# 30stomercury/whisper-char-alignment

Hardware: AMD Instinct MI355X
Metric: utterances/sec (whisper-medium, 10s audio, char align) at 1/2/4/8 MI355X (higher is better)
Workload: dtype f16x2 (hi + lo operand pairs on the f16 MFMA pipe: fp32-equivalent operands, fp32 accumulate)

## Files before the change

### whisper-char-alignment_amd/csrc/attention_split.hip

```cpp
#include <cstdlib>

#include "attn_common.h"
#include "launch.h"

namespace wca {

namespace {

template <bool CAUSAL, bool CAPTURE>
__global__ __launch_bounds__(256, 2) void attn_split_kernel(AttnArgs a) {
  constexpr int NW = 4;
  extern __shared__ __attribute__((aligned(16))) char smem[];
  half_t* lds = reinterpret_cast<half_t*>(smem);
  const int tid = threadIdx.x;
  const int lane = tid & 63;
  const int wave = __builtin_amdgcn_readfirstlane(tid >> 6);
  const int fr = lane & 15, fg = lane >> 4;
  constexpr int QB = NW * 32;
  const int n_qt = (a.nq + QB - 1) / QB;
  const int lid = xcd_remap(blockIdx.x, n_qt * a.H * a.B);
  const int bh = lid / n_qt;
  const int b = bh / a.H, h = bh - b * a.H;
  const int q_blk = (lid - bh * n_qt) * QB;
  const int q_wave = q_blk + wave * 32;

  half8 qh[2][2], ql[2][2];
  int qrow[2];
#pragma unroll
  for (int sub = 0; sub < 2; ++sub) {
    qrow[sub] = q_wave + sub * 16 + fr;
    const int qc = qrow[sub] < a.nq ? qrow[sub] : a.nq - 1;
    const half_t* qp = a.Q + (long)b * a.q_bs + (long)qc * a.q_rs + h * 64 + fg * 8;
    qh[sub][0] = *reinterpret_cast<const half8*>(qp);
    qh[sub][1] = *reinterpret_cast<const half8*>(qp + 32);
    ql[sub][0] = *reinterpret_cast<const half8*>(qp + a.q_lo);
    ql[sub][1] = *reinterpret_cast<const half8*>(qp + a.q_lo + 32);
  }
  const float c_log2 = a.scale * LOG2E;
  constexpr bool PRE = !CAPTURE;
  if (PRE) {
#pragma unroll
    for (int sub = 0; sub < 2; ++sub)
#pragma unroll
      for (int ks = 0; ks < 2; ++ks)
#pragma unroll
        for (int j = 0; j < 8; ++j) {
          const HalfPair pr = split_pair(((float)qh[sub][ks][j] + (float)ql[sub][ks][j]) * c_log2);
          qh[sub][ks][j] = pr.hi;
          ql[sub][ks][j] = pr.lo;
        }
  }
  const float cm = PRE ? 1.0f : c_log2;

  int nk_eff = a.nk;
  if (CAUSAL) {
    const int qhi = q_blk + QB;
    nk_eff = qhi < a.nk ? qhi : a.nk;
  }
  const int nkt = (nk_eff + KT - 1) / KT;

  const half_t* Kb = a.K + (long)b * a.k_bs + h * 64;
  const half_t* Vb = a.V + (long)b * a.v_bs + h * 64;

  auto stage = [&](int buf, int kt) {
    half_t* Kh = lds + buf * (4 * TILE);
    half_t* Kl = Kh + TILE;
    half_t* Vh = Kl + TILE;
    half_t* Vl = Vh + TILE;
#pragma unroll
    for (int i = 0; i < (8 + NW - 1) / NW; ++i) {
      const int piece = wave + NW * i;
      if (piece >= 8) break;
      const int rbase = piece * 8;
      const int r = rbase + (lane >> 3);
      int key = kt * KT + r;
      key = key < a.nk ? key : a.nk - 1;
      const int ck = (lane & 7) ^ swz128(r);
      const int cv = (lane & 7) ^ (r & 6);
      const half_t* kp = Kb + (long)key * a.k_rs + ck * 8;
      const half_t* vp = Vb + (long)key * a.v_rs + cv * 8;
      glds16(kp, Kh + rbase * 64);
      glds16(kp + a.k_lo, Kl + rbase * 64);
      glds16(vp, Vh + rbase * 64);
      glds16(vp + a.v_lo, Vl + rbase * 64);
    }
  };

  f32x4 ot[2][4];
#pragma unroll
  for (int s = 0; s < 2; ++s)
#pragma unroll
    for (int d = 0; d < 4; ++d) ot[s][d] = f32x4{0.f, 0.f, 0.f, 0.f};
  unsigned vaddr[4];
  {
    const int qd = fr >> 2, pd = fr & 3;
    const int swz = (4 * (fg & 1)) | (qd & 2);
#pragma unroll
    for (int dt = 0; dt < 4; ++dt)
      vaddr[dt] = lds_off(lds) + 2u * (unsigned)((4 * fg + qd) * 64 + (((2 * dt + (pd >> 1)) ^ swz) << 3) + 4 * (pd & 1));
  }
  unsigned kaddr[2][4];
#pragma unroll
  for (int ks = 0; ks < 2; ++ks)
#pragma unroll
    for (int t = 0; t < 4; ++t) {
      const int r = t * 16 + fr;
      kaddr[ks][t] = lds_off(lds) + 2u * (unsigned)(r * 64 + (((ks * 4 + fg) ^ swz128(r)) << 3));
    }
  float m_run[2] = {-INFINITY, -INFINITY};
  float l_part[2] = {0.f, 0.f};

  stage(0, 0);
  for (int kt = 0; kt < nkt; ++kt) {
    wait_vm0();
    __builtin_amdgcn_s_barrier();
    asm volatile("" ::: "memory");
    if (kt + 1 < nkt) stage((kt + 1) & 1, kt + 1);
    f32x4 st[2][4];
#pragma unroll
    for (int s = 0; s < 2; ++s)
#pragma unroll
      for (int t = 0; t < 4; ++t) st[s][t] = f32x4{0.f, 0.f, 0.f, 0.f};
    {
      constexpr int KLO = TILE * (int)sizeof(half_t);
      const unsigned sbk = (unsigned)(kt & 1) * (unsigned)(4 * TILE * sizeof(half_t));
      half8 kh[2][4], kl[2][4];
#pragma unroll
      for (int ks = 0; ks < 2; ++ks) {
#pragma unroll
        for (int t = 0; t < 4; ++t) kl[ks][t] = lds_read_b128_asm<KLO>(kaddr[ks][t] + sbk);
#pragma unroll
        for (int t = 0; t < 4; ++t) kh[ks][t] = lds_read_b128_asm<0>(kaddr[ks][t] + sbk);
      }
      WCA_LGKM_WAIT4(12, kl[0][0], kl[0][1], kl[0][2], kl[0][3]);
#pragma unroll
      for (int s = 0; s < 2; ++s)
#pragma unroll
        for (int t = 0; t < 4; ++t) st[s][t] = __builtin_amdgcn_mfma_f32_16x16x32_f16(kl[0][t], qh[s][0], st[s][t], 0, 0, 0);
      WCA_LGKM_WAIT4(8, kh[0][0], kh[0][1], kh[0][2], kh[0][3]);
#pragma unroll
      for (int s = 0; s < 2; ++s)
#pragma unroll
        for (int t = 0; t < 4; ++t) st[s][t] = __builtin_amdgcn_mfma_f32_16x16x32_f16(kh[0][t], ql[s][0], st[s][t], 0, 0, 0);
#pragma unroll
      for (int s = 0; s < 2; ++s)
#pragma unroll
        for (int t = 0; t < 4; ++t) st[s][t] = __builtin_amdgcn_mfma_f32_16x16x32_f16(kh[0][t], qh[s][0], st[s][t], 0, 0, 0);
      WCA_LGKM_WAIT4(4, kl[1][0], kl[1][1], kl[1][2], kl[1][3]);
#pragma unroll
      for (int s = 0; s < 2; ++s)
#pragma unroll
        for (int t = 0; t < 4; ++t) st[s][t] = __builtin_amdgcn_mfma_f32_16x16x32_f16(kl[1][t], qh[s][1], st[s][t], 0, 0, 0);
      WCA_LGKM_WAIT4(0, kh[1][0], kh[1][1], kh[1][2], kh[1][3]);
#pragma unroll
      for (int s = 0; s < 2; ++s)
#pragma unroll
        for (int t = 0; t < 4; ++t) st[s][t] = __builtin_amdgcn_mfma_f32_16x16x32_f16(kh[1][t], ql[s][1], st[s][t], 0, 0, 0);
#pragma unroll
      for (int s = 0; s < 2; ++s)
#pragma unroll
        for (int t = 0; t < 4; ++t) st[s][t] = __builtin_amdgcn_mfma_f32_16x16x32_f16(kh[1][t], qh[s][1], st[s][t], 0, 0, 0);
    }

    if (CAPTURE) {
#pragma unroll
      for (int s = 0; s < 2; ++s) {
        if (qrow[s] < a.nq) {
#pragma unroll
          for (int t = 0; t < 4; ++t) {
            const int key4 = kt * KT + t * 16 + 4 * fg;
            if (key4 < a.cap_cols) {
              float* cp = a.cap + (long)b * a.cap_bs + (long)h * a.cap_hs + (long)qrow[s] * a.cap_ld + key4;
              const f32x4 lg = st[s][t] * a.scale;
              if (key4 + 4 <= a.cap_cols) {
                *reinterpret_cast<f32x4*>(cp) = lg;
              } else {
#pragma unroll
                for (int r = 0; r < 3; ++r)
                  if (key4 + r < a.cap_cols) cp[r] = lg[r];
              }
            }
          }
        }
      }
    }
    const bool tail_tile = (kt * KT + KT > a.nk);
    const bool diag_tile = CAUSAL && (kt * KT + KT - 1 > q_wave);
    if (tail_tile || diag_tile) {
#pragma unroll
      for (int s = 0; s < 2; ++s)
#pragma unroll
        for (int t = 0; t < 4; ++t)
#pragma unroll
          for (int r = 0; r < 4; ++r) {
            const int key = kt * KT + t * 16 + 4 * fg + r;
            bool dead = key >= a.nk;
            if (CAUSAL) dead = dead || (key > qrow[s]);
            st[s][t][r] = dead ? -INFINITY : st[s][t][r];
          }
    }
    float mx[2];
#pragma unroll
    for (int s = 0; s < 2; ++s) {
      float m = fmaxf(fmaxf(st[s][0][0], st[s][0][1]), fmaxf(st[s][0][2], st[s][0][3]));
#pragma unroll
      for (int t = 1; t < 4; ++t) {
        m = fmaxf(fmaxf(m, st[s][t][0]), st[s][t][1]);
        m = fmaxf(fmaxf(m, st[s][t][2]), st[s][t][3]);
      }
      mx[s] = xor32_max(xor16_max(m));
    }
    const float thr_raw = 8.0f / cm;
    if (__any((mx[0] > m_run[0] + thr_raw) || (mx[1] > m_run[1] + thr_raw) || (m_run[0] == -INFINITY && mx[0] != -INFINITY) ||
              (m_run[1] == -INFINITY && mx[1] != -INFINITY))) {
#pragma unroll
      for (int s = 0; s < 2; ++s) {
        const float m_new = fmaxf(m_run[s], mx[s]);
        const float alpha = (m_run[s] == -INFINITY) ? 1.0f : __builtin_amdgcn_exp2f((m_run[s] - m_new) * cm);
        l_part[s] *= alpha;
#pragma unroll
        for (int d = 0; d < 4; ++d) ot[s][d] *= alpha;
        m_run[s] = m_new;
      }
    }
    half8 ph[2][2], pl[2][2];
#pragma unroll
    for (int s = 0; s < 2; ++s) {
      const float mref = (m_run[s] == -INFINITY) ? 0.f : m_run[s];
      const f32x2 mm = f32x2{mref, mref};
      f32x2 psum2 = f32x2{0.f, 0.f};
#pragma unroll
      for (int k2 = 0; k2 < 2; ++k2) {
        half2_ hh[4], ll[4];
#pragma unroll
        for (int u = 0; u < 4; ++u) {
          const int t = 2 * k2 + (u >> 1), r0 = 2 * (u & 1);
          f32x2 x = f32x2{st[s][t][r0], st[s][t][r0 + 1]} - mm;
          if (!PRE) x = x * f32x2{cm, cm};
          const f32x2 p = f32x2{__builtin_amdgcn_exp2f(x[0]), __builtin_amdgcn_exp2f(x[1])};
          psum2 += p;
          hh[u] = __builtin_convertvector(p, half2_);
          {
            const unsigned hu = __builtin_bit_cast(unsigned, hh[u]);
            unsigned lu;
            asm("v_fma_mixlo_f16 %0, %1, 1.0, -%2 op_sel:[0,0,0] op_sel_hi:[0,0,1]" : "=v"(lu) : "v"(p[0]), "v"(hu));
            asm("v_fma_mixhi_f16 %0, %1, 1.0, -%2 op_sel:[0,0,1] op_sel_hi:[0,0,1]" : "+v"(lu) : "v"(p[1]), "v"(hu));
            ll[u] = __builtin_bit_cast(half2_, lu);
          }
        }
        ph[s][k2] = half8{hh[0][0], hh[0][1], hh[1][0], hh[1][1], hh[2][0], hh[2][1], hh[3][0], hh[3][1]};
        pl[s][k2] = half8{ll[0][0], ll[0][1], ll[1][0], ll[1][1], ll[2][0], ll[2][1], ll[3][0], ll[3][1]};
      }
      l_part[s] += psum2[0] + psum2[1];
    }

    {
      const unsigned sb = (unsigned)(kt & 1) * (unsigned)(4 * TILE * sizeof(half_t));
      constexpr int VH = 2 * TILE * (int)sizeof(half_t), VL = 3 * TILE * (int)sizeof(half_t);
      constexpr int K2 = 32 * 64 * (int)sizeof(half_t), B16 = 16 * 64 * (int)sizeof(half_t);
      half4 c_[8], n_[8];
#define WCA_ISSUE_V(R, A)                                                                    \
  do {                                                                                       \
    R[0] = lds_read_tr_asm<VH>(A);                                                               \
    R[1] = lds_read_tr_asm<VH + B16>(A);                                                         \
    R[2] = lds_read_tr_asm<VL>(A);                                                               \
    R[3] = lds_read_tr_asm<VL + B16>(A);                                                         \
    R[4] = lds_read_tr_asm<VH + K2>(A);                                                          \
    R[5] = lds_read_tr_asm<VH + K2 + B16>(A);                                                    \
    R[6] = lds_read_tr_asm<VL + K2>(A);                                                          \
    R[7] = lds_read_tr_asm<VL + K2 + B16>(A);                                                    \
  } while (0)
      WCA_ISSUE_V(c_, vaddr[0] + sb);
#pragma unroll
      for (int dt = 0; dt < 4; ++dt) {
        if (dt < 3) {
          WCA_ISSUE_V(n_, vaddr[dt + 1] + sb);
          WCA_LGKM_WAIT8(8, c_[0], c_[1], c_[2], c_[3], c_[4], c_[5], c_[6], c_[7]);
        } else {
          WCA_LGKM_WAIT8(0, c_[0], c_[1], c_[2], c_[3], c_[4], c_[5], c_[6], c_[7]);
        }
#pragma unroll
        for (int k2 = 0; k2 < 2; ++k2) {
          const half8 vh = __builtin_shufflevector(c_[4 * k2], c_[4 * k2 + 1], 0, 1, 2, 3, 4, 5, 6, 7);
          const half8 vl = __builtin_shufflevector(c_[4 * k2 + 2], c_[4 * k2 + 3], 0, 1, 2, 3, 4, 5, 6, 7);
#pragma unroll
          for (int s = 0; s < 2; ++s) {
            ot[s][dt] = __builtin_amdgcn_mfma_f32_16x16x32_f16(vl, ph[s][k2], ot[s][dt], 0, 0, 0);
            ot[s][dt] = __builtin_amdgcn_mfma_f32_16x16x32_f16(vh, pl[s][k2], ot[s][dt], 0, 0, 0);
            ot[s][dt] = __builtin_amdgcn_mfma_f32_16x16x32_f16(vh, ph[s][k2], ot[s][dt], 0, 0, 0);
          }
        }
        if (dt < 3) {
#pragma unroll
          for (int i = 0; i < 8; ++i) c_[i] = n_[i];
        }
      }
#undef WCA_ISSUE_V
    }
  }

#pragma unroll
  for (int s = 0; s < 2; ++s) {
    const float l = xor32_sum(xor16_sum(l_part[s]));
    if (qrow[s] >= a.nq) continue;
    const float inv = 1.0f / l;
    half_t* op = a.O + (long)b * a.o_bs + (long)qrow[s] * a.o_rs + h * 64 + 4 * fg;
#pragma unroll
    for (int dt = 0; dt < 4; ++dt) {
      half4 oh, ol;
#pragma unroll
      for (int r = 0; r < 4; ++r) {
        const HalfPair pr = split_pair(ot[s][dt][r] * inv);
        oh[r] = pr.hi;
        ol[r] = pr.lo;
      }
      *reinterpret_cast<half4*>(op + dt * 16) = oh;
      *reinterpret_cast<half4*>(op + a.o_lo + dt * 16) = ol;
    }
  }
}



#define WCA_S_PIN8(A, B, C, D, E, F, G, H) asm volatile("" : "+v"(A), "+v"(B), "+v"(C), "+v"(D), "+v"(E), "+v"(F), "+v"(G), "+v"(H)::"memory")

template <int DROP>
__global__ __launch_bounds__(256, 2) void attn_split32_kernel(AttnArgs a) {
  constexpr int NW = 4;
  extern __shared__ __attribute__((aligned(16))) char smem[];
  half_t* lds = reinterpret_cast<half_t*>(smem);
  const int tid = threadIdx.x;
  const int lane = tid & 63;
  const int wave = __builtin_amdgcn_readfirstlane(tid >> 6);
  const int l31 = lane & 31, hh = lane >> 5;
  constexpr int QB = NW * 32;
  constexpr int TB = TILE * (int)sizeof(half_t);
  constexpr int SLOT_BYTES = 4 * TB;
  const int n_qt = (a.nq + QB - 1) / QB;
  const int lid = xcd_remap(blockIdx.x, n_qt * a.H * a.B);
  const int bh = lid / n_qt;
  const int b = bh / a.H, h = bh - b * a.H;
  const int q_wave = (lid - bh * n_qt) * QB + wave * 32;
  const int qrow = q_wave + l31;
  const float c_log2 = a.scale * LOG2E;
  half8 qh[4], ql[4];
  {
    const int qc = qrow < a.nq ? qrow : a.nq - 1;
    const half_t* qp = a.Q + (long)b * a.q_bs + (long)qc * a.q_rs + h * 64 + hh * 8;
#pragma unroll
    for (int ks = 0; ks < 4; ++ks) {
      const half8 rh = *reinterpret_cast<const half8*>(qp + ks * 16);
      const half8 rl = *reinterpret_cast<const half8*>(qp + a.q_lo + ks * 16);
#pragma unroll
      for (int j = 0; j < 8; ++j) {
        const HalfPair pr = split_pair(((float)rh[j] + (float)rl[j]) * c_log2);
        qh[ks][j] = pr.hi;
        ql[ks][j] = pr.lo;
      }
    }
  }
  const int nkt = (a.nk + KT - 1) / KT;
  const int kbytes = (int)(((long)(a.nk - 1) * a.k_rs + 64) * 2), vbytes = (int)(((long)(a.nk - 1) * a.v_rs + 64) * 2);
  const half_t* Kb = a.K + (long)b * a.k_bs + h * 64;
  const half_t* Vb = a.V + (long)b * a.v_bs + h * 64;
  const __amdgpu_buffer_rsrc_t rkh = __builtin_amdgcn_make_buffer_rsrc(const_cast<half_t*>(Kb), 0, kbytes, 0x00020000);
  const __amdgpu_buffer_rsrc_t rkl = __builtin_amdgcn_make_buffer_rsrc(const_cast<half_t*>(Kb + a.k_lo), 0, kbytes, 0x00020000);
  const __amdgpu_buffer_rsrc_t rvh = __builtin_amdgcn_make_buffer_rsrc(const_cast<half_t*>(Vb), 0, vbytes, 0x00020000);
  const __amdgpu_buffer_rsrc_t rvl = __builtin_amdgcn_make_buffer_rsrc(const_cast<half_t*>(Vb + a.v_lo), 0, vbytes, 0x00020000);
  unsigned dk[2], dv[2];
#pragma unroll
  for (int i = 0; i < 2; ++i) {
    const int r = (wave * 2 + i) * 8 + (lane >> 3);
    dk[i] = (unsigned)(r * a.k_rs * 2 + (((lane & 7) ^ ((r >> 1) & 7)) << 4));
    dv[i] = (unsigned)(r * a.v_rs * 2 + (((lane & 7) ^ ((r & 2) << 1)) << 4));
  }
  const unsigned k_tile_bytes = (unsigned)(KT * a.k_rs * 2), v_tile_bytes = (unsigned)(KT * a.v_rs * 2);
  auto stage = [&](int buf, int kt) {
    half_t* Kh = lds + buf * (4 * TILE);
#pragma unroll
    for (int i = 0; i < 2; ++i) {
      const int rbase = (wave * 2 + i) * 8;
      __builtin_amdgcn_raw_ptr_buffer_load_lds(rkh, (WCA_LDS void*)(Kh + rbase * 64), 16, (int)dk[i], (int)(kt * k_tile_bytes), 0, 0);
      __builtin_amdgcn_raw_ptr_buffer_load_lds(rkl, (WCA_LDS void*)(Kh + TILE + rbase * 64), 16, (int)dk[i], (int)(kt * k_tile_bytes), 0, 0);
      __builtin_amdgcn_raw_ptr_buffer_load_lds(rvh, (WCA_LDS void*)(Kh + 2 * TILE + rbase * 64), 16, (int)dv[i], (int)(kt * v_tile_bytes), 0, 0);
      __builtin_amdgcn_raw_ptr_buffer_load_lds(rvl, (WCA_LDS void*)(Kh + 3 * TILE + rbase * 64), 16, (int)dv[i], (int)(kt * v_tile_bytes), 0, 0);
    }
  };

  const int kswz = (l31 >> 1) & 7;
  const unsigned lds_base = lds_off(lds);
  unsigned ka[4];
#pragma unroll
  for (int ks = 0; ks < 4; ++ks) ka[ks] = lds_base + (unsigned)(l31 * 128 + 16 * ((hh ^ kswz) & 1) + 32 * (ks ^ (kswz >> 1)));
  const int vq = (lane & 15) >> 2, vp = lane & 3, vg1 = (lane >> 4) & 1;
  const int vkey0 = 4 * hh + vq;
  const int vdim0 = 16 * vg1 + 4 * vp;
  const int vsw = (vkey0 & 2) << 1;
  unsigned va[2];
#pragma unroll
  for (int db = 0; db < 2; ++db)
    va[db] = lds_base + (unsigned)(2 * TB + vkey0 * 128 + (((4 * db + (vdim0 >> 3)) ^ vsw) << 4) + 2 * (vdim0 & 7));

  f32x16 ot[2];
#pragma unroll
  for (int d = 0; d < 2; ++d)
#pragma unroll
    for (int r = 0; r < 16; ++r) ot[d][r] = 0.f;
  float m_run = -INFINITY;
  float l_run = 0.f;
  f32x16 cinit;
#pragma unroll
  for (int r = 0; r < 16; ++r) cinit[r] = 0.f;

  stage(0, 0);
  auto tile = [&](auto slot_c, int kt) {
    constexpr int SLOT = decltype(slot_c)::value;
    constexpr int SB = SLOT * SLOT_BYTES;
    asm volatile("s_waitcnt vmcnt(0)" ::: "memory");
    __builtin_amdgcn_s_barrier();
    asm volatile("" ::: "memory");
    if (kt + 1 < nkt) stage(SLOT ^ 1, kt + 1);

    f32x16 st[2];
    {
      half8 kl0[4], kh0[4], kl1[4], kh1[4];
      kl0[0] = lds_read_b128_asm<SB + TB>(ka[0]);
      kl0[1] = lds_read_b128_asm<SB + TB>(ka[1]);
      kl0[2] = lds_read_b128_asm<SB + TB>(ka[2]);
      kl0[3] = lds_read_b128_asm<SB + TB>(ka[3]);
      kh0[0] = lds_read_b128_asm<SB>(ka[0]);
      kh0[1] = lds_read_b128_asm<SB>(ka[1]);
      kh0[2] = lds_read_b128_asm<SB>(ka[2]);
      kh0[3] = lds_read_b128_asm<SB>(ka[3]);
      kl1[0] = lds_read_b128_asm<SB + TB + 32 * 128>(ka[0]);
      kl1[1] = lds_read_b128_asm<SB + TB + 32 * 128>(ka[1]);
      kl1[2] = lds_read_b128_asm<SB + TB + 32 * 128>(ka[2]);
      kl1[3] = lds_read_b128_asm<SB + TB + 32 * 128>(ka[3]);
      kh1[0] = lds_read_b128_asm<SB + 32 * 128>(ka[0]);
      kh1[1] = lds_read_b128_asm<SB + 32 * 128>(ka[1]);
      kh1[2] = lds_read_b128_asm<SB + 32 * 128>(ka[2]);
      kh1[3] = lds_read_b128_asm<SB + 32 * 128>(ka[3]);
      if constexpr (DROP == 0) {
      WCA_LGKM_WAIT4(12, kl0[0], kl0[1], kl0[2], kl0[3]);
      st[0] = __builtin_amdgcn_mfma_f32_32x32x16_f16(kl0[0], qh[0], cinit, 0, 0, 0);
#pragma unroll
      for (int ks = 1; ks < 4; ++ks) st[0] = __builtin_amdgcn_mfma_f32_32x32x16_f16(kl0[ks], qh[ks], st[0], 0, 0, 0);
      WCA_LGKM_WAIT4(8, kh0[0], kh0[1], kh0[2], kh0[3]);
#pragma unroll
      for (int ks = 0; ks < 4; ++ks) st[0] = __builtin_amdgcn_mfma_f32_32x32x16_f16(kh0[ks], ql[ks], st[0], 0, 0, 0);
#pragma unroll
      for (int ks = 0; ks < 4; ++ks) st[0] = __builtin_amdgcn_mfma_f32_32x32x16_f16(kh0[ks], qh[ks], st[0], 0, 0, 0);
      WCA_LGKM_WAIT4(4, kl1[0], kl1[1], kl1[2], kl1[3]);
// ... 37 lines not shown
    P##hb[1] = lds_read_tr_asm<SB + 1 * 2048 + 1024>(va[DB]);              \
    P##ha[2] = lds_read_tr_asm<SB + 2 * 2048>(va[DB]);                     \
    P##hb[2] = lds_read_tr_asm<SB + 2 * 2048 + 1024>(va[DB]);              \
    P##ha[3] = lds_read_tr_asm<SB + 3 * 2048>(va[DB]);                     \
    P##hb[3] = lds_read_tr_asm<SB + 3 * 2048 + 1024>(va[DB]);              \
    P##la[0] = lds_read_tr_asm<SB + TB + 0 * 2048>(va[DB]);                \
    P##lb[0] = lds_read_tr_asm<SB + TB + 0 * 2048 + 1024>(va[DB]);         \
    P##la[1] = lds_read_tr_asm<SB + TB + 1 * 2048>(va[DB]);                \
    P##lb[1] = lds_read_tr_asm<SB + TB + 1 * 2048 + 1024>(va[DB]);         \
    P##la[2] = lds_read_tr_asm<SB + TB + 2 * 2048>(va[DB]);                \
    P##lb[2] = lds_read_tr_asm<SB + TB + 2 * 2048 + 1024>(va[DB]);         \
    P##la[3] = lds_read_tr_asm<SB + TB + 3 * 2048>(va[DB]);                \
    P##lb[3] = lds_read_tr_asm<SB + TB + 3 * 2048 + 1024>(va[DB]);         \
  } while (0)
    WCA_ISSUE_V32(v0, 0);
    if (kt * KT + KT > a.nk) {
#pragma unroll
      for (int kb = 0; kb < 2; ++kb)
#pragma unroll
        for (int r = 0; r < 16; ++r) {
          const int key = kt * KT + kb * 32 + (r & 3) + 8 * (r >> 2) + 4 * hh;
          st[kb][r] = key >= a.nk ? -INFINITY : st[kb][r];
        }
    }
    float mx;
    {
      float m0 = max3f(st[0][0], st[0][1], st[0][2]), m1 = max3f(st[0][3], st[0][4], st[0][5]);
      float m2 = max3f(st[0][6], st[0][7], st[0][8]), m3 = max3f(st[0][9], st[0][10], st[0][11]);
      m0 = max3f(m0, st[0][12], st[0][13]);
      m1 = max3f(m1, st[0][14], st[0][15]);
      m2 = max3f(m2, st[1][0], st[1][1]);
      m3 = max3f(m3, st[1][2], st[1][3]);
      m0 = max3f(m0, st[1][4], st[1][5]);
      m1 = max3f(m1, st[1][6], st[1][7]);
      m2 = max3f(m2, st[1][8], st[1][9]);
      m3 = max3f(m3, st[1][10], st[1][11]);
      m0 = max3f(m0, st[1][12], st[1][13]);
      m1 = max3f(m1, st[1][14], st[1][15]);
      mx = fmaxf(max3f(m0, m1, m2), m3);
      mx = xor32_max(mx);
    }
    if (__any((mx > RESCALE_THR) || (m_run == -INFINITY && mx != -INFINITY))) {
      const float m_eff = (m_run == -INFINITY) ? 0.f : m_run;
      const float m_new = fmaxf(m_run, mx + m_eff);
      const float delta = (m_new == -INFINITY) ? 0.f : m_new - m_eff;
      const float alpha = (m_run == -INFINITY) ? 1.0f : __builtin_amdgcn_exp2f(m_run - m_new);
      l_run *= alpha;
#pragma unroll
      for (int d = 0; d < 2; ++d)
#pragma unroll
        for (int r = 0; r < 16; ++r) ot[d][r] *= alpha;
#pragma unroll
      for (int kb = 0; kb < 2; ++kb)
#pragma unroll
        for (int r = 0; r < 16; ++r) st[kb][r] -= delta;
      m_run = m_new;
      const float c0 = (m_new != -INFINITY) ? -m_new : 0.f;
#pragma unroll
      for (int r = 0; r < 16; ++r) cinit[r] = c0;
    }
    half8 ph[4], pl[4];
    {
      f32x2 psum = f32x2{0.f, 0.f};
#pragma unroll
      for (int s4 = 0; s4 < 4; ++s4) {
        half2_ hq[4], lq[4];
#pragma unroll
        for (int u = 0; u < 4; ++u) {
          const int r0 = 8 * (s4 & 1) + 2 * u;
          const f32x2 p = f32x2{__builtin_amdgcn_exp2f(st[s4 >> 1][r0]), __builtin_amdgcn_exp2f(st[s4 >> 1][r0 + 1])};
          psum += p;
          hq[u] = __builtin_convertvector(p, half2_);
          const unsigned hu = __builtin_bit_cast(unsigned, hq[u]);
          unsigned lu;
          asm("v_fma_mixlo_f16 %0, %1, 1.0, -%2 op_sel:[0,0,0] op_sel_hi:[0,0,1]" : "=v"(lu) : "v"(p[0]), "v"(hu));
          asm("v_fma_mixhi_f16 %0, %1, 1.0, -%2 op_sel:[0,0,1] op_sel_hi:[0,0,1]" : "+v"(lu) : "v"(p[1]), "v"(hu));
          lq[u] = __builtin_bit_cast(half2_, lu);
        }
        ph[s4] = half8{hq[0][0], hq[0][1], hq[1][0], hq[1][1], hq[2][0], hq[2][1], hq[3][0], hq[3][1]};
        pl[s4] = half8{lq[0][0], lq[0][1], lq[1][0], lq[1][1], lq[2][0], lq[2][1], lq[3][0], lq[3][1]};
      }
      l_run += psum[0] + psum[1];
    }
    WCA_LGKM_WAIT8(0, v0ha[0], v0hb[0], v0ha[1], v0hb[1], v0ha[2], v0hb[2], v0ha[3], v0hb[3]);
    WCA_S_PIN8(v0la[0], v0lb[0], v0la[1], v0lb[1], v0la[2], v0lb[2], v0la[3], v0lb[3]);
    WCA_ISSUE_V32(v1, 1);
#pragma unroll
    for (int s4 = 0; s4 < 4; ++s4) {
      const half8 wh = __builtin_shufflevector(v0ha[s4], v0hb[s4], 0, 1, 2, 3, 4, 5, 6, 7);
      const half8 wl = __builtin_shufflevector(v0la[s4], v0lb[s4], 0, 1, 2, 3, 4, 5, 6, 7);
      if (!(DROP & 4)) ot[0] = __builtin_amdgcn_mfma_f32_32x32x16_f16(wl, ph[s4], ot[0], 0, 0, 0);
      if (!(DROP & 8)) ot[0] = __builtin_amdgcn_mfma_f32_32x32x16_f16(wh, pl[s4], ot[0], 0, 0, 0);
      ot[0] = __builtin_amdgcn_mfma_f32_32x32x16_f16(wh, ph[s4], ot[0], 0, 0, 0);
    }
    WCA_LGKM_WAIT8(0, v1ha[0], v1hb[0], v1ha[1], v1hb[1], v1ha[2], v1hb[2], v1ha[3], v1hb[3]);
    WCA_S_PIN8(v1la[0], v1lb[0], v1la[1], v1lb[1], v1la[2], v1lb[2], v1la[3], v1lb[3]);
#pragma unroll
    for (int s4 = 0; s4 < 4; ++s4) {
      const half8 wh = __builtin_shufflevector(v1ha[s4], v1hb[s4], 0, 1, 2, 3, 4, 5, 6, 7);
      const half8 wl = __builtin_shufflevector(v1la[s4], v1lb[s4], 0, 1, 2, 3, 4, 5, 6, 7);
      if (!(DROP & 4)) ot[1] = __builtin_amdgcn_mfma_f32_32x32x16_f16(wl, ph[s4], ot[1], 0, 0, 0);
      if (!(DROP & 8)) ot[1] = __builtin_amdgcn_mfma_f32_32x32x16_f16(wh, pl[s4], ot[1], 0, 0, 0);
      ot[1] = __builtin_amdgcn_mfma_f32_32x32x16_f16(wh, ph[s4], ot[1], 0, 0, 0);
    }
#undef WCA_ISSUE_V32
  };
  for (int kt = 0; kt < nkt; kt += 2) {
    tile(IntC<0>{}, kt);
    if (kt + 1 < nkt) tile(IntC<1>{}, kt + 1);
  }

  const float inv = 1.0f / xor32_sum(l_run);
  half_t* op = a.O + (long)b * a.o_bs + (long)qrow * a.o_rs + h * 64;
#pragma unroll
  for (int db = 0; db < 2; ++db)
#pragma unroll
    for (int g2 = 0; g2 < 2; ++g2) {
      unsigned wh[2][2], wl[2][2];
#pragma unroll
      for (int e = 0; e < 2; ++e)
#pragma unroll
        for (int k2 = 0; k2 < 2; ++k2) {
          const Half2Pair pr = split_pair2(ot[db][4 * (2 * g2 + e) + 2 * k2] * inv, ot[db][4 * (2 * g2 + e) + 2 * k2 + 1] * inv);
          wh[e][k2] = __builtin_bit_cast(unsigned, pr.hi);
          wl[e][k2] = __builtin_bit_cast(unsigned, pr.lo);
        }
      typedef unsigned u32x4 __attribute__((ext_vector_type(4)));
      u32x4 oh, ol;
      {
        auto r0 = __builtin_amdgcn_permlane32_swap(wh[0][0], wh[1][0], false, false);
        auto r1 = __builtin_amdgcn_permlane32_swap(wh[0][1], wh[1][1], false, false);
        oh = u32x4{r0[0], r1[0], r0[1], r1[1]};
        auto s0 = __builtin_amdgcn_permlane32_swap(wl[0][0], wl[1][0], false, false);
        auto s1 = __builtin_amdgcn_permlane32_swap(wl[0][1], wl[1][1], false, false);
        ol = u32x4{s0[0], s1[0], s0[1], s1[1]};
      }
      if (qrow < a.nq) {
        *reinterpret_cast<u32x4*>(op + 32 * db + 16 * g2 + 8 * hh) = oh;
        *reinterpret_cast<u32x4*>(op + a.o_lo + 32 * db + 16 * g2 + 8 * hh) = ol;
      }
    }
}

}

hipError_t launch_attention_split(const AttnArgs& a, hipStream_t s) {
  if (a.nq <= 0 || a.B <= 0) return hipSuccess;
  if (!attn_args_ok(a)) return hipErrorInvalidValue;
  if ((a.q_lo % 8) || (a.k_lo % 8) || (a.v_lo % 8) || (a.o_lo % 4) || a.q_lo <= 0 || a.k_lo <= 0 || a.v_lo <= 0 || a.o_lo <= 0) return hipErrorInvalidValue;
  const bool cap = a.cap != nullptr && a.cap_cols > 0;
  constexpr int LDS = 2 * 4 * TILE * (int)sizeof(half_t);
  const dim3 grid(((a.nq + 127) / 128) * a.H * a.B), block(256);
  const int variant = a.variant ? a.variant : debug_switch(DBG_ATTN_SPLIT_VARIANT);
  if (!a.causal && !cap && a.nq >= 64 && variant != 1 && (a.o_rs % 8) == 0 && (a.o_lo % 8) == 0) {
    auto launch32 = [&](auto drop_c) { return launch_lds<attn_split32_kernel<decltype(drop_c)::value>, LDS>(grid, block, LDS, s, a); };
    switch (debug_switch(DBG_ATTN_SPLIT_DROP)) {
      case 0: return launch32(IntC<0>{});
      case 1: return launch32(IntC<1>{});
      case 2: return launch32(IntC<2>{});
      case 3: return launch32(IntC<3>{});
      case 4: return launch32(IntC<4>{});
      case 8: return launch32(IntC<8>{});
      case 9: return launch32(IntC<9>{});
      case 12: return launch32(IntC<12>{});
      case 15: return launch32(IntC<15>{});
      default: return hipErrorInvalidValue;
    }
  }
  if (a.causal) {
    if (cap) return launch_lds<attn_split_kernel<true, true>, LDS>(grid, block, LDS, s, a);
    return launch_lds<attn_split_kernel<true, false>, LDS>(grid, block, LDS, s, a);
  }
  if (cap) return launch_lds<attn_split_kernel<false, true>, LDS>(grid, block, LDS, s, a);
  return launch_lds<attn_split_kernel<false, false>, LDS>(grid, block, LDS, s, a);
}

}
```

### whisper-char-alignment_amd/csrc/engine_forward.hip

```cpp
#include "engine_internal.h"

using namespace wca;

namespace wca {

hipError_t gemm(wca_engine* e, hipStream_t s, Gemm g) {
  if (g.c_lo > 0 && g.out_mode == 0) g.out_mode = 4;
  if (g.w_plain != nullptr && use_wlo(e) && e->wlo_bases.count(g.w_plain)) {
    GemmArgs x = flat(g.A, g.lda, g.w_lo ? g.w_lo : wlo_of(e, g.w_plain), g.k_plain, g.C, g.ldc, g.M, g.N, g.k_plain);
    x.a_rows_per_batch = g.a_rows_per_batch;
    x.a_batch_stride = g.a_batch_stride;
    x.site = g.site;
    x.out_mode = 2;
    if (g.out_mode != 2) {
      GrowBuf& tmp = e->wlo_tmp[s == e->stream ? 0 : 1];
      if (hipError_t he = tmp.ensure((size_t)g.M * g.N * sizeof(float)); he != hipSuccess) return he;
      x.C = tmp.p;
      x.ldc = g.N;
      x.out_mode = 1;
      g.addend = (const float*)tmp.p;
      g.ld_addend = g.N;
    }
    if (hipError_t he = launch_gemm(x, s); he != hipSuccess) return he;
  }
// ... 190 lines not shown
  Gemm g = flat(e->xn, sp, e->kv_w, e->sw.kv_w, d, kvbuf, (sp ? 2 : 1) * L * 2 * dt, B * N_CTX, n_cols);
  g.bias = e->kv_b;
  g.c_lo = sp ? (long)L * 2 * dt : 0;
  g.site = 3;
  HIPCHK(gemm(e, e->stream, g));
  return WCA_OK;
}

struct DecPass {
  hipStream_t s;
  int B, nq;
  bool pair;
  const half_t* kv;
  int kv_group;
  half_t* cache;
  int T_max;
  StepPos pos;
  const int* nk_rows() const { return pos.rows ? pos.rows + B : nullptr; }
  half_t* scatter;
  float* cap;
  int Fpad, Fcap;
  int l0, l1;
  bool stop_at_capture;
};

namespace {

int dec_linear(wca_engine* e, const DecPass& p, Gemm g, const half_t* W2, half_t* xn) {
  if (!p.pair) return dec_gemm(e, p.s, g, xn);
  const bool f16_out = g.out_mode == 0;
  if (g.A32) {
    HIPCHK(launch_layernorm_f16(g.A32, g.ln_gamma, g.ln_beta, xn, g.M, g.K, 1e-5f, p.s, 2 * g.K, g.K));
    g.A = xn;
  }
  Gemm m = flat(g.A, true, g.W, W2, g.K, g.C, (f16_out ? 2 : 1) * g.ldc, g.M, g.N);
  m.bias = g.bias;
  m.gelu = g.gelu;
  m.out_mode = g.out_mode;
  m.site = g.site;
  m.c_lo = f16_out ? g.N : 0;
  m.sk_part = e->sk_big[1];
  m.sk_bytes = e->sk_big_bytes;
  HIPCHK(gemm(e, p.s, m));
  return WCA_OK;
}

Gemm dec_flat(const half_t* A, const half_t* W, const float* bias, void* C, int M, int N, int K) {
  Gemm g = flat(A, K, W, K, C, N, M, N, K);
  g.bias = bias;
  g.site = 2;
  return g;
}
Gemm dec_flat_ln(const float* x, const float* gamma, const float* beta, const half_t* W, const float* bias, void* C, int M, int N, int K) {
  Gemm g = flat(nullptr, 0, W, K, C, N, M, N, K);
  g.A32 = x;
  g.ln_gamma = gamma;
  g.ln_beta = beta;
  g.bias = bias;
  g.site = 2;
  return g;
}

AttnArgs attn_common(const wca_engine* e, const DecPass& p, const half_t* q, int q_rs, half_t* o) {
  const int dt = e->dims.n_text_state, H = e->dims.n_text_head, om = p.pair ? 2 : 1;
  AttnArgs a{};
  a.Q = q;
  a.q_bs = (long)p.nq * q_rs;
  a.q_rs = q_rs;
  a.O = o;
  a.o_bs = (long)p.nq * om * dt;
  a.o_rs = om * dt;
  if (p.pair) {
    a.split = 1;
    a.o_lo = dt;
  }
  a.nq = p.nq;
  a.H = H;
  a.B = p.B;
  a.scale = 1.0f / std::sqrt((float)(dt / H));
  return a;
}

AttnArgs self_attn_args(const wca_engine* e, const DecPass& p, const half_t* qkv, half_t* o, const half_t* kc, const half_t* vc) {
  const int dt = e->dims.n_text_state, om = p.pair ? 2 : 1;
  AttnArgs a = attn_common(e, p, qkv, om * 3 * dt, o);
  if (p.cache) {
    a.K = kc;
    a.V = vc;
    a.k_bs = a.v_bs = (long)p.T_max * dt;
    a.k_rs = a.v_rs = dt;
    a.nk = p.pos.rows ? p.T_max : p.pos.t + 1;
    a.nk_rows = p.nk_rows();
    return a;
  }
  a.K = qkv + dt;
  a.V = qkv + 2 * dt;
  a.k_bs = a.v_bs = a.q_bs;
  a.k_rs = a.v_rs = a.q_rs;
  if (p.pair) a.q_lo = a.k_lo = a.v_lo = 3 * dt;
  a.nk = p.nq;
  a.causal = 1;
  return a;
}

AttnArgs cross_attn_args(const wca_engine* e, const DecPass& p, int li, const half_t* q, half_t* o) {
  const int dt = e->dims.n_text_state, H = e->dims.n_text_head, L = e->dims.n_text_layer, om = p.pair ? 2 : 1;
  const int kv_ld = (e->split ? 2 : 1) * L * 2 * dt;
  AttnArgs a = attn_common(e, p, q, om * dt, o);
  a.K = p.kv + (size_t)(2 * li) * dt;
  a.V = p.kv + (size_t)(2 * li + 1) * dt;
  a.k_bs = a.v_bs = (long)N_CTX * kv_ld;
  a.k_rs = a.v_rs = kv_ld;
  if (p.pair) {
    a.q_lo = dt;
    a.k_lo = a.v_lo = (long)L * 2 * dt;
  }
  a.cap = p.cap ? p.cap + (size_t)li * H * p.nq * p.Fpad : nullptr;
  a.cap_bs = (long)L * H * p.nq * p.Fpad;
  a.cap_hs = (long)p.nq * p.Fpad;
  a.cap_ld = p.Fpad;
  a.cap_cols = p.Fcap;
  a.nk = N_CTX;
  a.kv_group = p.kv_group;
  return a;
}

int run_decoder_layers(wca_engine* e, const DecPass& p) {
  const int dt = e->dims.n_text_state, L = e->dims.n_text_layer;
  const int M = p.B * p.nq;
  float* xd = e->xd;
  half_t *xdn = e->xdn, *qkv_d = e->qkv_d, *att_d = e->att_d, *q_d = e->q_d, *hid_d = e->hid_d;
  half_t* planes = p.cache ? p.cache : p.scatter;
  const size_t plane = (size_t)p.B * p.T_max * dt;
  for (int li = p.l0; li < p.l1; ++li) {
    const LayerW& l = e->dec[li];
    const LayerW& w2 = p.pair ? e->sw.dec[li] : l;
    half_t* kc = planes ? planes + (size_t)(2 * li) * plane : nullptr;
    half_t* vc = planes ? kc + plane : nullptr;
    Gemm g = dec_flat_ln(xd, l.ln1_g, l.ln1_b, l.qkv_w, l.qkv_b, qkv_d, M, 3 * dt, dt);
    if (p.cache) {
      g.kv_k = kc;
      g.kv_v = vc;
      g.kv_tmax = p.T_max;
      g.kv_t = p.pos.t;
      g.kv_t_rows = p.pos.rows;
    }
    WCA_TRY(dec_linear(e, p, g, w2.qkv_w, xdn));
    if (p.scatter) HIPCHK(launch_kv_scatter(qkv_d, kc, vc, p.B, p.nq, p.T_max, dt, p.s));
    HIPCHK(launch_attention(self_attn_args(e, p, qkv_d, att_d, kc, vc), p.s));
    g = dec_flat(att_d, l.out_w, l.out_b, xd, M, dt, dt);
    g.out_mode = 2;
    WCA_TRY(dec_linear(e, p, g, w2.out_w, xdn));
    WCA_TRY(dec_linear(e, p, dec_flat_ln(xd, l.lnc_g, l.lnc_b, l.cq_w, l.cq_b, q_d, M, dt, dt), w2.cq_w, xdn));
    HIPCHK(launch_attention(cross_attn_args(e, p, li, q_d, att_d), p.s));
    if (li == L - 1 && p.stop_at_capture) break;
    g = dec_flat(att_d, l.co_w, l.co_b, xd, M, dt, dt);
    g.out_mode = 2;
    WCA_TRY(dec_linear(e, p, g, w2.co_w, xdn));
    g = dec_flat_ln(xd, l.ln2_g, l.ln2_b, l.fc1_w, l.fc1_b, hid_d, M, 4 * dt, dt);
    g.gelu = 1;
    WCA_TRY(dec_linear(e, p, g, w2.fc1_w, xdn));
    g = dec_flat(hid_d, l.fc2_w, l.fc2_b, xd, M, dt, 4 * dt);
    g.out_mode = 2;
    WCA_TRY(dec_linear(e, p, g, w2.fc2_w, xdn));
  }
  return WCA_OK;
}

int dec_logits(wca_engine* e, const DecPass& p, const float* x, half_t* xn, int M, float* logits) {
  const wca_model_dims& D = e->dims;
  Gemm g = dec_flat_ln(x, e->lnf_g, e->lnf_b, e->tok_emb, nullptr, logits, M, D.n_vocab, D.n_text_state);
  g.out_mode = 1;
  g.site = 3;
  return dec_linear(e, p, g, e->sw.tok_emb, xn);
}

}

int run_decoder(wca_engine* e, const int64_t* tokens_dev, int B, int n, float* cap, int Fpad, int Fcap, float* logits_out, hipStream_t s,
                const half_t* kvbuf, bool finish_last) {
  const wca_model_dims& D = e->dims;
  DecPass p{};
  p.s = s ? s : e->stream;
  p.B = B;
  p.nq = n;
  p.pair = e->split;
  p.kv = kvbuf ? kvbuf : e->kv;
  p.cap = cap;
  p.Fpad = Fpad;
  p.Fcap = Fcap;
  p.l1 = D.n_text_layer;
  p.stop_at_capture = !logits_out && !finish_last;
  HIPCHK(launch_embed(tokens_dev, e->tok_emb, e->dec_pos, e->xd, B, n, D.n_text_state, D.n_vocab, e->err_dev, p.s,
                      (e->split && use_wlo(e) && e->wlo_bases.count(e->tok_emb)) ? wlo_of(e, e->tok_emb) : nullptr));
  WCA_TRY(run_decoder_layers(e, p));
  if (logits_out) WCA_TRY(dec_logits(e, p, e->xd, e->xdn, B * n, logits_out));
  return WCA_OK;
}

int run_decode_step(wca_engine* e, hipStream_t s, const half_t* kvbuf, const int* tokens, int B, StepPos pos, int T_max, bool want_logits,
                    int kv_group) {
  const wca_model_dims& D = e->dims;
  DecPass p{};
  p.s = s;
  p.B = B;
  p.nq = 1;
  p.kv = kvbuf;
  p.kv_group = kv_group;
  p.cache = (half_t*)e->dec_cache.p + e->dec_cache_off;
  p.T_max = T_max;
  p.pos = pos;
  p.l1 = D.n_text_layer;
  HIPCHK(launch_embed_step(tokens, T_max, pos, e->tok_emb, e->dec_pos, e->xd, B, D.n_text_state, D.n_vocab, s));
  WCA_TRY(run_decoder_layers(e, p));
  if (want_logits) WCA_TRY(dec_logits(e, p, e->xd, e->xdn, B, (float*)e->dec_logits.p));
  return WCA_OK;
}

int run_decode_prefill(wca_engine* e, hipStream_t s, const half_t* kvbuf, const int* tokens, int B, int n, int T_max, StepPos last, StepPos sot) {
  const int dt = e->dims.n_text_state;
  DecPass p{};
  p.s = s;
  p.B = B;
  p.nq = n;
  p.kv = kvbuf;
  p.scatter = (half_t*)e->dec_cache.p + e->dec_cache_off;
  p.T_max = T_max;
  p.l1 = e->dims.n_text_layer;
  HIPCHK(launch_embed_prefix(tokens, T_max, n, e->tok_emb, e->dec_pos, e->xd, B, dt, e->dims.n_vocab, s));
  WCA_TRY(run_decoder_layers(e, p));
  const int R = ((last.rows ? sot.rows != nullptr : sot.t >= 0) ? 2 : 1) * B;
  float* xg = (float*)e->dec_gather.p;
  HIPCHK(launch_gather_rows(e->xd, xg, B, n, last, sot, dt, s));
  return dec_logits(e, p, xg, e->xdn, R, (float*)e->dec_logits.p);
}

}

namespace {

__global__ void mel_to_tm_kernel(const float* __restrict__ mel, half_t* __restrict__ tm, int n_mels, int B, int row, int lo_off) {
  const int b = blockIdx.y;
  const long e0 = (long)blockIdx.x * blockDim.x + threadIdx.x;
  if (e0 >= (long)n_mels * N_FRAMES) return;
  const int t = (int)(e0 / n_mels), m = (int)(e0 - (long)t * n_mels);
  const float v = mel[((long)b * n_mels + m) * N_FRAMES + t];
  const half_t hv = (half_t)v;
  half_t* o = tm + ((long)b * (N_FRAMES + 2) + t + 1) * row + m;
  o[0] = hv;
  if (lo_off) o[lo_off] = (half_t)(v - (float)hv);
}

}

namespace wca {

int mel_to_tm(wca_engine* e, const float* mel_dev, int batch) {
  const wca_model_dims& D = e->dims;
  const size_t nel = (size_t)D.n_mels * N_FRAMES;
  dim3 grid((unsigned)((nel + 255) / 256), batch);
  hipLaunchKernelGGL(mel_to_tm_kernel, grid, dim3(256), 0, e->stream, mel_dev, e->mel_tm, D.n_mels, batch, (e->split ? 2 : 1) * D.n_mels, e->split ? D.n_mels : 0);
  HIPCHK(hipGetLastError());
  return WCA_OK;
}

int run_phase1(wca_engine* e, const float* mel_dev, const float* pcm_dev, int64_t pcm_stride, const int* n_samples_dev, int batch, int slot,
               bool skip_last_v) {
  half_t* kvbuf = slot ? e->kv_alt : e->kv;
  record(e, 0);
  if (pcm_dev) {
    int rc = run_logmel(e, pcm_dev, pcm_stride, n_samples_dev, batch, nullptr, true);
    if (rc) return rc;
  } else {
    if (int mr = mel_to_tm(e, mel_dev, batch)) return mr;
  }
  record(e, 1);
  e->ln_err = e->err_dev + 1 + slot;
  HIPCHK(hipMemsetAsync(e->ln_err, 0, sizeof(int), e->stream));
  int rc = run_encoder(e, batch);
  e->ln_err = e->err_dev;
  if (!rc) {
    record(e, 2);
    rc = run_cross_kv(e, batch, kvbuf, skip_last_v);
  }
  if (rc) return rc;
  record(e, 3);
  HIPCHK(hipEventRecord(e->ev_kv[slot], e->stream));
  return WCA_OK;
}

}
```

Baseline: 335.1.

## Add few-query cross-attention variant and capture-only path skipping unused PV work

Adds a templated few-query form of the split attention kernel for cross-attention with logit capture. Waves whose query rows fall past nq now skip their MFMA work, or run a single sub-tile. When the last decoder layer stops at capture, the attention output is not needed, so a capture-only instantiation skips V staging, softmax and the PV product. This removes redundant V loads and MFMAs at the cost of more template instantiations and a new null-output contract.

```diff
diff --git a/whisper-char-alignment_amd/csrc/attention_split.hip b/whisper-char-alignment_amd/csrc/attention_split.hip
--- a/whisper-char-alignment_amd/csrc/attention_split.hip
+++ b/whisper-char-alignment_amd/csrc/attention_split.hip
@@ -7,9 +7,13 @@
 
 namespace {
 
-template <bool CAUSAL, bool CAPTURE>
+template <bool CAUSAL, bool CAPTURE, bool FEW = false, bool PV = true>
 __global__ __launch_bounds__(256, 2) void attn_split_kernel(AttnArgs a) {
+  static_assert(!FEW || (CAPTURE && !CAUSAL), "the few-query form is the cross-attention with capture");
+  static_assert(PV || FEW, "only the few-query form has a capture-only call");
   constexpr int NW = 4;
+  constexpr int SLOT = (PV ? 4 : 2) * TILE;
+  constexpr unsigned SLOT_BYTES = SLOT * sizeof(half_t);
   extern __shared__ __attribute__((aligned(16))) char smem[];
   half_t* lds = reinterpret_cast<half_t*>(smem);
   const int tid = threadIdx.x;
@@ -60,10 +64,10 @@
   const int nkt = (nk_eff + KT - 1) / KT;
 
   const half_t* Kb = a.K + (long)b * a.k_bs + h * 64;
-  const half_t* Vb = a.V + (long)b * a.v_bs + h * 64;
+  const half_t* Vb = PV ? a.V + (long)b * a.v_bs + h * 64 : nullptr;
 
   auto stage = [&](int buf, int kt) {
-    half_t* Kh = lds + buf * (4 * TILE);
+    half_t* Kh = lds + buf * SLOT;
     half_t* Kl = Kh + TILE;
     half_t* Vh = Kl + TILE;
     half_t* Vl = Vh + TILE;
@@ -78,11 +82,13 @@
       const int ck = (lane & 7) ^ swz128(r);
       const int cv = (lane & 7) ^ (r & 6);
       const half_t* kp = Kb + (long)key * a.k_rs + ck * 8;
-      const half_t* vp = Vb + (long)key * a.v_rs + cv * 8;
       glds16(kp, Kh + rbase * 64);
       glds16(kp + a.k_lo, Kl + rbase * 64);
-      glds16(vp, Vh + rbase * 64);
-      glds16(vp + a.v_lo, Vl + rbase * 64);
+      if constexpr (PV) {
+        const half_t* vp = Vb + (long)key * a.v_rs + cv * 8;
+        glds16(vp, Vh + rbase * 64);
+        glds16(vp + a.v_lo, Vl + rbase * 64);
+      }
     }
   };
 
@@ -110,20 +116,16 @@
   float m_run[2] = {-INFINITY, -INFINITY};
   float l_part[2] = {0.f, 0.f};
 
-  stage(0, 0);
-  for (int kt = 0; kt < nkt; ++kt) {
-    wait_vm0();
-    __builtin_amdgcn_s_barrier();
-    asm volatile("" ::: "memory");
-    if (kt + 1 < nkt) stage((kt + 1) & 1, kt + 1);
+  auto tile = [&](auto nsub_c, int kt) {
+    constexpr int NSUB = decltype(nsub_c)::value;
     f32x4 st[2][4];
 #pragma unroll
-    for (int s = 0; s < 2; ++s)
+    for (int s = 0; s < NSUB; ++s)
 #pragma unroll
       for (int t = 0; t < 4; ++t) st[s][t] = f32x4{0.f, 0.f, 0.f, 0.f};
     {
       constexpr int KLO = TILE * (int)sizeof(half_t);
-      const unsigned sbk = (unsigned)(kt & 1) * (unsigned)(4 * TILE * sizeof(half_t));
+      const unsigned sbk = (unsigned)(kt & 1) * SLOT_BYTES;
       half8 kh[2][4], kl[2][4];
 #pragma unroll
       for (int ks = 0; ks < 2; ++ks) {
@@ -134,37 +136,37 @@
       }
       WCA_LGKM_WAIT4(12, kl[0][0], kl[0][1], kl[0][2], kl[0][3]);
 #pragma unroll
-      for (int s = 0; s < 2; ++s)
+      for (int s = 0; s < NSUB; ++s)
 #pragma unroll
         for (int t = 0; t < 4; ++t) st[s][t] = __builtin_amdgcn_mfma_f32_16x16x32_f16(kl[0][t], qh[s][0], st[s][t], 0, 0, 0);
       WCA_LGKM_WAIT4(8, kh[0][0], kh[0][1], kh[0][2], kh[0][3]);
 #pragma unroll
-      for (int s = 0; s < 2; ++s)
+      for (int s = 0; s < NSUB; ++s)
 #pragma unroll
         for (int t = 0; t < 4; ++t) st[s][t] = __builtin_amdgcn_mfma_f32_16x16x32_f16(kh[0][t], ql[s][0], st[s][t], 0, 0, 0);
 #pragma unroll
-      for (int s = 0; s < 2; ++s)
+      for (int s = 0; s < NSUB; ++s)
 #pragma unroll
         for (int t = 0; t < 4; ++t) st[s][t] = __builtin_amdgcn_mfma_f32_16x16x32_f16(kh[0][t], qh[s][0], st[s][t], 0, 0, 0);
       WCA_LGKM_WAIT4(4, kl[1][0], kl[1][1], kl[1][2], kl[1][3]);
 #pragma unroll
-      for (int s = 0; s < 2; ++s)
+      for (int s = 0; s < NSUB; ++s)
 #pragma unroll
         for (int t = 0; t < 4; ++t) st[s][t] = __builtin_amdgcn_mfma_f32_16x16x32_f16(kl[1][t], qh[s][1], st[s][t], 0, 0, 0);
       WCA_LGKM_WAIT4(0, kh[1][0], kh[1][1], kh[1][2], kh[1][3]);
 #pragma unroll
-      for (int s = 0; s < 2; ++s)
+      for (int s = 0; s < NSUB; ++s)
 #pragma unroll
         for (int t = 0; t < 4; ++t) st[s][t] = __builtin_amdgcn_mfma_f32_16x16x32_f16(kh[1][t], ql[s][1], st[s][t], 0, 0, 0);
 #pragma unroll
-      for (int s = 0; s < 2; ++s)
+      for (int s = 0; s < NSUB; ++s)
 #pragma unroll
         for (int t = 0; t < 4; ++t) st[s][t] = __builtin_amdgcn_mfma_f32_16x16x32_f16(kh[1][t], qh[s][1], st[s][t], 0, 0, 0);
     }
 
     if (CAPTURE) {
 #pragma unroll
-      for (int s = 0; s < 2; ++s) {
+      for (int s = 0; s < NSUB; ++s) {
         if (qrow[s] < a.nq) {
 #pragma unroll
           for (int t = 0; t < 4; ++t) {
@@ -184,11 +186,12 @@
         }
       }
     }
+    if constexpr (PV) {
     const bool tail_tile = (kt * KT + KT > a.nk);
     const bool diag_tile = CAUSAL && (kt * KT + KT - 1 > q_wave);
     if (tail_tile || diag_tile) {
 #pragma unroll
-      for (int s = 0; s < 2; ++s)
+      for (int s = 0; s < NSUB; ++s)
 #pragma unroll
         for (int t = 0; t < 4; ++t)
 #pragma unroll
@@ -201,7 +204,7 @@
     }
     float mx[2];
 #pragma unroll
-    for (int s = 0; s < 2; ++s) {
+    for (int s = 0; s < NSUB; ++s) {
       float m = fmaxf(fmaxf(st[s][0][0], st[s][0][1]), fmaxf(st[s][0][2], st[s][0][3]));
 #pragma unroll
       for (int t = 1; t < 4; ++t) {
@@ -211,10 +214,11 @@
       mx[s] = xor32_max(xor16_max(m));
     }
     const float thr_raw = 8.0f / cm;
-    if (__any((mx[0] > m_run[0] + thr_raw) || (mx[1] > m_run[1] + thr_raw) || (m_run[0] == -INFINITY && mx[0] != -INFINITY) ||
-              (m_run[1] == -INFINITY && mx[1] != -INFINITY))) {
-#pragma unroll
-      for (int s = 0; s < 2; ++s) {
+    bool raise = (mx[0] > m_run[0] + thr_raw) || (m_run[0] == -INFINITY && mx[0] != -INFINITY);
+    if (NSUB == 2) raise = raise || (mx[1] > m_run[1] + thr_raw) || (m_run[1] == -INFINITY && mx[1] != -INFINITY);
+    if (__any(raise)) {
+#pragma unroll
+      for (int s = 0; s < NSUB; ++s) {
         const float m_new = fmaxf(m_run[s], mx[s]);
         const float alpha = (m_run[s] == -INFINITY) ? 1.0f : __builtin_amdgcn_exp2f((m_run[s] - m_new) * cm);
         l_part[s] *= alpha;
@@ -225,7 +229,7 @@
     }
     half8 ph[2][2], pl[2][2];
 #pragma unroll
-    for (int s = 0; s < 2; ++s) {
+    for (int s = 0; s < NSUB; ++s) {
       const float mref = (m_run[s] == -INFINITY) ? 0.f : m_run[s];
       const f32x2 mm = f32x2{mref, mref};
       f32x2 psum2 = f32x2{0.f, 0.f};
@@ -255,7 +259,7 @@
     }
 
     {
-      const unsigned sb = (unsigned)(kt & 1) * (unsigned)(4 * TILE * sizeof(half_t));
+      const unsigned sb = (unsigned)(kt & 1) * SLOT_BYTES;
       constexpr int VH = 2 * TILE * (int)sizeof(half_t), VL = 3 * TILE * (int)sizeof(half_t);
       constexpr int K2 = 32 * 64 * (int)sizeof(half_t), B16 = 16 * 64 * (int)sizeof(half_t);
       half4 c_[8], n_[8];
@@ -284,7 +288,7 @@
           const half8 vh = __builtin_shufflevector(c_[4 * k2], c_[4 * k2 + 1], 0, 1, 2, 3, 4, 5, 6, 7);
           const half8 vl = __builtin_shufflevector(c_[4 * k2 + 2], c_[4 * k2 + 3], 0, 1, 2, 3, 4, 5, 6, 7);
 #pragma unroll
-          for (int s = 0; s < 2; ++s) {
+          for (int s = 0; s < NSUB; ++s) {
             ot[s][dt] = __builtin_amdgcn_mfma_f32_16x16x32_f16(vl, ph[s][k2], ot[s][dt], 0, 0, 0);
             ot[s][dt] = __builtin_amdgcn_mfma_f32_16x16x32_f16(vh, pl[s][k2], ot[s][dt], 0, 0, 0);
             ot[s][dt] = __builtin_amdgcn_mfma_f32_16x16x32_f16(vh, ph[s][k2], ot[s][dt], 0, 0, 0);
@@ -297,7 +301,20 @@
       }
 #undef WCA_ISSUE_V
     }
-  }
+    }
+  };
+
+  const int nsub = !FEW || q_wave + 16 < a.nq ? 2 : (q_wave < a.nq ? 1 : 0);
+  stage(0, 0);
+  for (int kt = 0; kt < nkt; ++kt) {
+    wait_vm0();
+    __builtin_amdgcn_s_barrier();
+    asm volatile("" ::: "memory");
+    if (kt + 1 < nkt) stage((kt + 1) & 1, kt + 1);
+    if (nsub == 2) tile(IntC<2>{}, kt);
+    else if (nsub == 1) tile(IntC<1>{}, kt);
+  }
+  if (!PV || nsub == 0) return;
 
 #pragma unroll
   for (int s = 0; s < 2; ++s) {
@@ -641,6 +658,8 @@
   constexpr int LDS = 2 * 4 * TILE * (int)sizeof(half_t);
   const dim3 grid(((a.nq + 127) / 128) * a.H * a.B), block(256);
   const int variant = a.variant ? a.variant : debug_switch(DBG_ATTN_SPLIT_VARIANT);
+  const bool few = cap && !a.causal && a.nq <= 128 && (variant != 1 || a.O == nullptr);
+  if (a.O == nullptr && !few) return hipErrorInvalidValue;
   if (!a.causal && !cap && a.nq >= 64 && variant != 1 && (a.o_rs % 8) == 0 && (a.o_lo % 8) == 0) {
     auto launch32 = [&](auto drop_c) { return launch_lds<attn_split32_kernel<decltype(drop_c)::value>, LDS>(grid, block, LDS, s, a); };
     switch (debug_switch(DBG_ATTN_SPLIT_DROP)) {
@@ -656,6 +675,10 @@
       default: return hipErrorInvalidValue;
     }
   }
+  if (few) {
+    if (a.O == nullptr) return launch_lds<attn_split_kernel<false, true, true, false>, LDS>(grid, block, LDS, s, a);
+    return launch_lds<attn_split_kernel<false, true, true, true>, LDS>(grid, block, LDS, s, a);
+  }
   if (a.causal) {
     if (cap) return launch_lds<attn_split_kernel<true, true>, LDS>(grid, block, LDS, s, a);
     return launch_lds<attn_split_kernel<true, false>, LDS>(grid, block, LDS, s, a);
diff --git a/whisper-char-alignment_amd/csrc/engine_forward.hip b/whisper-char-alignment_amd/csrc/engine_forward.hip
--- a/whisper-char-alignment_amd/csrc/engine_forward.hip
+++ b/whisper-char-alignment_amd/csrc/engine_forward.hip
@@ -366,8 +366,10 @@
     g.out_mode = 2;
     WCA_TRY(dec_linear(e, p, g, w2.out_w, xdn));
     WCA_TRY(dec_linear(e, p, dec_flat_ln(xd, l.lnc_g, l.lnc_b, l.cq_w, l.cq_b, q_d, M, dt, dt), w2.cq_w, xdn));
-    HIPCHK(launch_attention(cross_attn_args(e, p, li, q_d, att_d), p.s));
-    if (li == L - 1 && p.stop_at_capture) break;
+    const bool last_stop = li == L - 1 && p.stop_at_capture;
+    const bool cap_only = last_stop && p.pair && p.cap != nullptr && p.Fcap > 0 && p.nq <= 128;
+    HIPCHK(launch_attention(cross_attn_args(e, p, li, q_d, cap_only ? nullptr : att_d), p.s));
+    if (last_stop) break;
     g = dec_flat(att_d, l.co_w, l.co_b, xd, M, dt, dt);
     g.out_mode = 2;
     WCA_TRY(dec_linear(e, p, g, w2.co_w, xdn));
```

New measurement: 336.2, median of 2. About the same (+0.3%).
